# malak29/video-text-detection-system

Measured on AMD Instinct MI355X. Metric: frames/sec (detect+recognize) @720p, 1/2/4/8 MI355X; box IoU vs CPU ref, higher is better.
Workload: dtype f16

## Files before the change

video-text-detection-system_amd/csrc/conv_halo.hip:

```cpp
#include <cstdio>
#include <cstdlib>
#include "vtd_common.h"
#include "conv_kernels.h"

namespace {

struct HaloParams {
    const half_t* in;
    const half_t* wgt;
    const float* bias;
    const half_t* res;
    half_t* out;
    int n, h, w, cin, cout;
    int in_hp, in_wp, in_ring, out_hp, out_wp, out_ring, res_hp, res_wp, res_ring;
    int tiles_x, tiles_y, tiles_n, relu;
    unsigned long long* stamps;
    const half_t* in2 = nullptr;
    int in2_hp = 0, in2_wp = 0, in2_c = 0, in2_ring = 0;
    int K = 0;
    int dbg;
};

template <int N>
__device__ __forceinline__ void hl_wait_vmcnt() {
    asm volatile("s_waitcnt vmcnt(%0)" ::"n"(N) : "memory");
}

template <int BN, int TW>
__global__ __launch_bounds__((BN / 64) * 256) void conv_halo_kernel(const HaloParams p) {
    constexpr int WN = BN / 64, NW = 4 * WN, NT = NW * 64, TH = 256 / TW;
    constexpr int HWD = TW + 2, HROWS = (TH + 2) * HWD, HPIECES = (HROWS + 7) / 8, HBYTES = HPIECES * 1024;
    constexpr int HPW = (HPIECES + NW - 1) / NW;
    constexpr int HPS = (HPW + 7) / 8;
    constexpr int BSTAGE = BN * 128, BPW = BN / 8 / NW;
    constexpr int EPI_ROW = BN * 4 + 16;
    static_assert(BPW == 2, "two weight pieces per wave and K-step");
    extern __shared__ __attribute__((aligned(16))) char smem[];

    const int nchunks = p.cin >> 6;
    const int hb_stride = nchunks > 1 ? HBYTES : 0;
    char* const bring = smem + (nchunks > 1 ? 2 : 1) * HBYTES;

    const int nblk = gridDim.x, b = blockIdx.x;
    const int q8 = nblk >> 3, r8 = nblk & 7, xcd = b & 7;
    int tile = (xcd < r8 ? xcd * (q8 + 1) : r8 * (q8 + 1) + (xcd - r8) * q8) + (b >> 3);
    const int tn = tile % p.tiles_n;
    tile /= p.tiles_n;
    const int tx = tile % p.tiles_x;
    tile /= p.tiles_x;
    const int ty = tile % p.tiles_y;
    const int img = tile / p.tiles_y;
    const int y0 = ty * TH, x0 = tx * TW, n0 = tn * BN;

    const int tid = threadIdx.x, lane = tid & 63;
    const int w = __builtin_amdgcn_readfirstlane(tid >> 6);
    const int lrow = lane >> 3;
    const int K = 9 * p.cin;

    int hoff[HPW];
#pragma unroll
    for (int k = 0; k < HPW; ++k) {
        const int piece = w + k * NW;
        int row = piece * 8 + lrow;
        row = row < HROWS ? row : HROWS - 1;
        const int hy = row / HWD, hx = row - hy * HWD;
        int gy = y0 - 1 + hy + p.in_ring, gx = x0 - 1 + hx + p.in_ring;
        gy = gy < p.in_hp ? gy : p.in_hp - 1;
        gx = gx < p.in_wp ? gx : p.in_wp - 1;
        const int c_log = (lane & 7) ^ (row & 6);
        hoff[k] = ((img * p.in_hp + gy) * p.in_wp + gx) * p.cin + c_log * 8;
    }
    auto issue_halo = [&](int k, int chunk, int buf) {
        const int piece = w + k * NW;
        if (piece < HPIECES)
            __builtin_amdgcn_global_load_lds((const VTD_AS1 void*)(p.in + hoff[k] + chunk * 64),
                                             (VTD_AS3 void*)(smem + buf * hb_stride + piece * 1024), 16, 0, 0);
    };
    const half_t* bsrc[BPW];
// ... 489 lines not shown
    for (int i = 0; i < 4; ++i) bias4[i] = *(const floatx4*)(p.bias + fq * 16 + i * 4);
#pragma unroll
    for (int i = 0; i < 4; ++i) asm volatile("" : "+v"(bias4[i]));

    auto tile_coords = [&](int t, int& img, int& y0, int& x0) {
        img = t / tiles_per_img;
        const int r = t - img * tiles_per_img, ty = r / p.tiles_x;
        y0 = ty * TH;
        x0 = (r - ty * p.tiles_x) * TW;
    };
    int hrel[HPW];
    int hdst[HPW];
#pragma unroll
    for (int k = 0; k < HPW; ++k) {
        const int piece = w + 4 * k;
        int row = piece * 8 + lrow;
        row = row < HROWS ? row : HROWS - 1;
        const int hy = row / HWD, hx = row - hy * HWD;
        hrel[k] = (hy * p.in_wp + hx) * 64 + ((lane & 7) ^ (row & 6)) * 8;
        hdst[k] = piece < HPIECES ? WBYTES + piece * 1024 : WBYTES + 2 * HBYTES;
    }
    auto issue_halo = [&](int img, int y0, int x0, int buf) {
        const half_t* base = p.in + ((int64_t)(img * p.in_hp + y0 - 1 + p.in_ring) * p.in_wp + x0 - 1 + p.in_ring) * 64;
#pragma unroll
        for (int k = 0; k < HPW; ++k)
            __builtin_amdgcn_global_load_lds((const VTD_AS1 void*)(base + hrel[k]),
                                             (VTD_AS3 void*)(smem + hdst[k] + (w + 4 * k < HPIECES ? buf * HBYTES : 0)), 16, 0, 0);
    };
    int orel[4], rrel[4];
#pragma unroll
    for (int j = 0; j < 4; ++j) {
        const int m = w * 64 + j * 16 + fr;
        orel[j] = ((m / TW) * p.out_wp + (m % TW)) * 64 + fq * 16;
        rrel[j] = ((m / TW) * p.res_wp + (m % TW)) * 64 + fq * 16;
    }

    int hbase[4];
#pragma unroll
    for (int j = 0; j < 4; ++j) {
        const int m = w * 64 + j * 16 + fr;
        hbase[j] = (m / TW) * HWD + (m % TW);
    }
    const int bswz = (fr >> 1) & 7;

    auto load_res = [&](int img, int y0, int x0, half8 (&rv)[4][2]) {
        const half_t* rbase = p.res + ((int64_t)(img * p.res_hp + y0 + p.res_ring) * p.res_wp + x0 + p.res_ring) * 64;
#pragma unroll
        for (int j = 0; j < 4; ++j) {
            rv[j][0] = *(const half8*)(rbase + rrel[j]);
            rv[j][1] = *(const half8*)(rbase + rrel[j] + 8);
        }
    };

    int tile = blockIdx.x;
    if (tile >= total) return;
    int img, y0, x0;
    tile_coords(tile, img, y0, x0);
    issue_halo(img, y0, x0, 0);
    int cur = 0;
    unsigned long long acc_wait = 0, acc_loop = 0, acc_epi = 0, t_a = 0, t_b = 0, t_c = 0;
    for (; tile < total; tile += gridDim.x, cur ^= 1) {
        if (p.stamps) t_a = __builtin_amdgcn_s_memtime();
        const int ntile = tile + gridDim.x;
        int nimg = img, ny0 = y0, nx0 = x0;
        half8 rv[4][2];
        if (RES) load_res(img, y0, x0, rv);
        if (ntile < total) tile_coords(ntile, nimg, ny0, nx0);
        issue_halo(nimg, ny0, nx0, cur ^ 1);
        if (RES) hl_wait_vmcnt<HPW + 8>(); else hl_wait_vmcnt<HPW>();
        __builtin_amdgcn_s_barrier();
        if (p.stamps) t_b = __builtin_amdgcn_s_memtime();

        floatx4 acc[4][4];
#pragma unroll
        for (int i = 0; i < 4; ++i)
#pragma unroll
            for (int j = 0; j < 4; ++j) acc[i][j] = bias4[i];
        const char* hb = hbuf + cur * HBYTES;
        auto load_frags = [&](int hs, half8 (&af)[4], half8 (&bf)[4]) {
            const int tap = hs >> 1, kk = hs & 1;
            const int tapoff = (tap / 3) * HWD + (tap % 3);
#pragma unroll
            for (int j = 0; j < 4; ++j) {
                const int hrow = hbase[j] + tapoff;
                af[j] = *(const half8*)(hb + hrow * 128 + (((fq + 4 * kk) ^ (hrow & 6)) << 4));
            }
#pragma unroll
            for (int i = 0; i < 4; ++i) bf[i] = *(const half8*)(wl + tap * 8192 + (i * 16 + fr) * 128 + (((fq + 4 * kk) ^ bswz) << 4));
        };
        half8 fa[2][4], fb[2][4];
        load_frags(0, fa[0], fb[0]);
#pragma unroll
        for (int hs = 0; hs < 18; ++hs) {
            if (hs + 1 < 18) load_frags(hs + 1, fa[(hs + 1) & 1], fb[(hs + 1) & 1]);
#pragma unroll
            for (int i = 0; i < 4; ++i)
#pragma unroll
                for (int j = 0; j < 4; ++j)
                    acc[i][j] = __builtin_amdgcn_mfma_f32_16x16x32_f16(fb[hs & 1][i], fa[hs & 1][j], acc[i][j], 0, 0, 0);
            if (hs + 1 < 18) {
                __builtin_amdgcn_sched_group_barrier(0x100, 8, 0);
                __builtin_amdgcn_sched_group_barrier(0x008, 16, 0);
            }
            __builtin_amdgcn_sched_barrier(0);
        }

        if (p.stamps) {
            asm volatile("s_nop 0" ::"v"(acc[3][3][3]));
            t_c = __builtin_amdgcn_s_memtime();
        }
        half_t* obase = p.out + ((int64_t)(img * p.out_hp + y0 + p.out_ring) * p.out_wp + x0 + p.out_ring) * 64;
#pragma unroll
        for (int j = 0; j < 4; ++j)
#pragma unroll
            for (int h = 0; h < 2; ++h) {
                half8 hv;
#pragma unroll
                for (int k = 0; k < 8; ++k) {
                    float v = acc[2 * h + (k >> 2)][j][k & 3];
                    if (RES) v += (float)rv[j][h][k];
                    hv[k] = (half_t)(RELU ? fmaxf(v, 0.f) : v);
                }
                *(half8*)(obase + orel[j] + h * 8) = hv;
            }
        __builtin_amdgcn_s_barrier();
        img = nimg; y0 = ny0; x0 = nx0;
        if (p.stamps) {
            const unsigned long long t_d = __builtin_amdgcn_s_memtime();
            acc_wait += t_b - t_a; acc_loop += t_c - t_b; acc_epi += t_d - t_c;
        }
    }
    if (p.stamps && tid == 0) {
        unsigned long long* o = p.stamps + (int64_t)blockIdx.x * 4;
        o[0] = 0; o[1] = acc_wait; o[2] = acc_wait + acc_loop; o[3] = acc_wait + acc_loop + acc_epi;
    }
    hl_wait_vmcnt<0>();
}

template <int TW, bool RELU, bool RES>
__global__ __launch_bounds__(512, 1) void conv3x3_c64_duo_kernel(const HaloParams p) {
    constexpr int TH = 256 / TW, HWD = TW + 2, HROWS = (TH + 2) * HWD, HPIECES = (HROWS + 7) / 8, HBYTES = HPIECES * 1024;
    constexpr int HPW = (HPIECES + 3) / 4;
    constexpr int WBYTES = 9 * 64 * 128;
    extern __shared__ __attribute__((aligned(16))) char smem[];
    char* const wl = smem;
    char* const hbuf = smem + WBYTES;

    const int tid = threadIdx.x, lane = tid & 63;
    const int wv = __builtin_amdgcn_readfirstlane(tid >> 6);
    const int g = wv >> 2, w = wv & 3;
    const int lrow = lane >> 3, fr = lane & 15, fq = lane >> 4;
    const int tiles_per_img = p.tiles_x * p.tiles_y, total = p.n * tiles_per_img;

#pragma unroll
    for (int k = 0; k < 9; ++k) {
        const int piece = wv + 8 * k, tap = piece >> 3, row = (piece & 7) * 8 + lrow;
        const int c_log = (lane & 7) ^ ((row >> 1) & 7);
        const int cout = 16 * ((row & 15) >> 2) + 4 * (row >> 4) + (row & 3);
        __builtin_amdgcn_global_load_lds((const VTD_AS1 void*)(p.wgt + cout * 576 + tap * 64 + c_log * 8),
                                         (VTD_AS3 void*)(wl + piece * 1024), 16, 0, 0);
    }
    float* const bias_lds = (float*)(smem + WBYTES + 2 * HBYTES + 1024);
    if (tid < 64) bias_lds[tid] = p.bias[tid];

    auto tile_coords = [&](int t, int& img, int& y0, int& x0) {
        img = t / tiles_per_img;
        const int r = t - img * tiles_per_img, ty = r / p.tiles_x;
        y0 = ty * TH;
        x0 = (r - ty * p.tiles_x) * TW;
    };
    auto issue_halo = [&](int t) {
        int img, y0, x0;
        tile_coords(t, img, y0, x0);
        const half_t* base = p.in + ((int64_t)(img * p.in_hp + y0 - 1 + p.in_ring) * p.in_wp + x0 - 1 + p.in_ring) * 64;
#pragma unroll
        for (int k = 0; k < HPW; ++k) {
            const int piece = w + 4 * k;
            int row = piece * 8 + lrow;
            row = row < HROWS ? row : HROWS - 1;
            const int hy = row / HWD, hx = row - hy * HWD;
            const int hrel = (hy * p.in_wp + hx) * 64 + ((lane & 7) ^ (hx & 6)) * 8;
            const int hdst = piece < HPIECES ? WBYTES + g * HBYTES + piece * 1024 : WBYTES + 2 * HBYTES;
            __builtin_amdgcn_global_load_lds((const VTD_AS1 void*)(base + hrel), (VTD_AS3 void*)(smem + hdst), 16, 0, 0);
        }
    };
    auto px_row = [&](int j) { return (w * 64 + j * 16 + fr) / TW; };
    auto px_col = [&](int j) { return (w * 64 + j * 16 + fr) % TW; };
    const int a_lane_off = (px_row(0) * HWD + px_col(0)) * 128;
    const int b_lane_off = fr * 128;
    const int bswz = (fr >> 1) & 7;
    const char* const hb = hbuf + g * HBYTES;

    const int nq = (total - (int)blockIdx.x + (int)gridDim.x - 1) / (int)gridDim.x;
    const int nmine = (nq - g + 1) >> 1;
    const int phases = 2 * ((nq + 1) >> 1) > 2 * (nq >> 1) + 1 ? 2 * ((nq + 1) >> 1) : 2 * (nq >> 1) + 1;
#ifdef VTD_CONV_EXPERIMENT
    auto block_of = [&](int i) { return p.dbg == 1 ? (int)blockIdx.x : (int)blockIdx.x + (2 * i + g) * (int)gridDim.x; };
#else
    auto block_of = [&](int i) { return (int)blockIdx.x + (2 * i + g) * (int)gridDim.x; };
#endif

    if (nmine > 0) issue_halo(block_of(0));
    hl_wait_vmcnt<0>();
    asm volatile("s_waitcnt lgkmcnt(0)" ::: "memory");
    __builtin_amdgcn_s_barrier();

    floatx4 acc[4][4];
    half8 rv[4][2];
    for (int phase = 0; phase < phases; ++phase) {
        if ((phase & 1) == g) {
            const int i = (phase - g) >> 1;
            if (i < nmine) {
                if (RES) {
                    int img, y0, x0;
                    tile_coords(block_of(i), img, y0, x0);
                    const half_t* rbase = p.res + ((int64_t)(img * p.res_hp + y0 + p.res_ring) * p.res_wp + x0 + p.res_ring) * 64;
#pragma unroll
                    for (int j = 0; j < 4; ++j) {
                        const int rrel = (px_row(j) * p.res_wp + px_col(j)) * 64 + fq * 16;
                        rv[j][0] = *(const half8*)(rbase + rrel);
                        rv[j][1] = *(const half8*)(rbase + rrel + 8);
                    }
                }
#pragma unroll
                for (int a = 0; a < 4; ++a)
#pragma unroll
                    for (int j = 0; j < 4; ++j) acc[a][j] = *(const floatx4*)(bias_lds + fq * 16 + a * 4);
                auto load_frags = [&](int hs, half8 (&af)[4], half8 (&bf)[4]) {
                    const int tap = hs >> 1, kk = hs & 1;
                    const int tapoff = (tap / 3) * HWD + (tap % 3), dx = tap % 3;
                    const char* pa = hb + a_lane_off + tapoff * 128 + (((fq + 4 * kk) ^ ((fr + dx) & 6)) << 4);
                    const char* pb = wl + tap * 8192 + b_lane_off + (((fq + 4 * kk) ^ bswz) << 4);
#pragma unroll
                    for (int j = 0; j < 4; ++j) af[j] = *(const half8*)(pa + (TW == 16 ? j * HWD : (j >> 1) * HWD + (j & 1) * 16) * 128);
#pragma unroll
                    for (int a = 0; a < 4; ++a) bf[a] = *(const half8*)(pb + a * 2048);
                };
                half8 fa[2][4], fb[2][4];
                load_frags(0, fa[0], fb[0]);
#pragma unroll
                for (int hs = 0; hs < 18; ++hs) {
                    if (hs + 1 < 18) load_frags(hs + 1, fa[(hs + 1) & 1], fb[(hs + 1) & 1]);
#pragma unroll
                    for (int a = 0; a < 4; ++a)
#pragma unroll
                        for (int j = 0; j < 4; ++j)
                            acc[a][j] = __builtin_amdgcn_mfma_f32_16x16x32_f16(fb[hs & 1][a], fa[hs & 1][j], acc[a][j], 0, 0, 0);
                    if (hs + 1 < 18) {
                        __builtin_amdgcn_sched_group_barrier(0x100, 8, 0);
                        __builtin_amdgcn_sched_group_barrier(0x008, 16, 0);
                    }
                    __builtin_amdgcn_sched_barrier(0);
                    if (hs + 1 < 18) {
#pragma unroll
                        for (int j = 0; j < 4; ++j) asm volatile("" ::"v"(fa[(hs + 1) & 1][j]));
#pragma unroll
                        for (int a = 0; a < 4; ++a) asm volatile("" ::"v"(fb[(hs + 1) & 1][a]));
                    }
                }
            }
        } else {
            const int i = (phase - g - 1) >> 1;
            if (phase - g - 1 >= 0 && i < nmine) {
                if (i + 1 < nmine) issue_halo(block_of(i + 1));
                int img, y0, x0;
                tile_coords(block_of(i), img, y0, x0);
                half_t* obase = p.out + ((int64_t)(img * p.out_hp + y0 + p.out_ring) * p.out_wp + x0 + p.out_ring) * 64;
#pragma unroll
                for (int j = 0; j < 4; ++j)
#pragma unroll
                    for (int h = 0; h < 2; ++h) {
                        half8 hv;
#pragma unroll
                        for (int k = 0; k < 8; ++k) {
                            float v = acc[2 * h + (k >> 2)][j][k & 3];
                            if (RES) v += (float)rv[j][h][k];
                            hv[k] = (half_t)(RELU ? fmaxf(v, 0.f) : v);
                        }
                        *(half8*)(obase + (px_row(j) * p.out_wp + px_col(j)) * 64 + fq * 16 + h * 8) = hv;
                    }
            }
            hl_wait_vmcnt<0>();
        }
        __builtin_amdgcn_s_barrier();
    }
    hl_wait_vmcnt<0>();
}

template <int TW, bool RELU, bool RES>
int c64_launch(const HaloParams& p, hipStream_t stream) {
    constexpr int TH = 256 / TW, HROWS = (TH + 2) * (TW + 2), HBYTES = (HROWS + 7) / 8 * 1024;
    constexpr int lds = 9 * 64 * 128 + 2 * HBYTES + 1024 + 256;
    static_assert(lds <= 160 * 1024, "LDS budget");
    if (p.h % TH || p.w % TW) return -2205;
    static bool attr_done = false;
    if (!attr_done) {
        hipError_t e = hipFuncSetAttribute((const void*)conv3x3_c64_persistent_kernel<TW, RELU, RES>,
                                           hipFuncAttributeMaxDynamicSharedMemorySize, lds);
        if (e != hipSuccess) return -(int)e;
        attr_done = true;
    }
    const int total = p.n * p.tiles_y * p.tiles_x;
    const int grid = total < 256 ? total : 256;
    static const bool want_stamps = [] { const char* e = getenv("VTD_HALO_STAMPS"); return e && e[0] == '1'; }();
    if (want_stamps) {
        HaloParams q = p;
        unsigned long long* dev = nullptr;
        if (hipMalloc(&dev, (size_t)grid * 32) != hipSuccess) return -2204;
        q.stamps = dev;
        hipLaunchKernelGGL((conv3x3_c64_persistent_kernel<TW, RELU, RES>), dim3(grid), dim3(256), lds, stream, q);
        (void)hipStreamSynchronize(stream);
        unsigned long long* h = (unsigned long long*)malloc((size_t)grid * 32);
        (void)hipMemcpy(h, dev, (size_t)grid * 32, hipMemcpyDeviceToHost);
        double a = 0, b = 0, c = 0;
        for (int i = 0; i < grid; ++i) { a += (double)h[4 * i + 1]; b += (double)(h[4 * i + 2] - h[4 * i + 1]); c += (double)(h[4 * i + 3] - h[4 * i + 2]); }
        const double blocks = (double)total / grid;
        fprintf(stderr, "[c64 stamps] res=%d blocks/WG %.1f: per block ticks: issue+wait %.1f  K-loop %.1f  epilogue %.1f\n", (int)RES, blocks,
                a / grid / blocks, b / grid / blocks, c / grid / blocks);
        free(h);
        (void)hipFree(dev);
        return 0;
    }
    const char* duo_env = getenv("VTD_C64_DUO");
    const bool duo = !(duo_env && duo_env[0] == '0');
#ifdef VTD_CONV_EXPERIMENT
    if (duo) {
        HaloParams q = p;
        const char* d = getenv("VTD_C64_DEBUG");
        q.dbg = d ? atoi(d) : 0;
        hipError_t e = hipFuncSetAttribute((const void*)conv3x3_c64_duo_kernel<TW, RELU, RES>, hipFuncAttributeMaxDynamicSharedMemorySize, lds);
        if (e != hipSuccess) return -(int)e;
        hipLaunchKernelGGL((conv3x3_c64_duo_kernel<TW, RELU, RES>), dim3(grid), dim3(512), lds, stream, q);
        return -(int)hipGetLastError();
    }
#endif
    if (duo) {
        static bool attr_duo = false;
        if (!attr_duo) {
            hipError_t e = hipFuncSetAttribute((const void*)conv3x3_c64_duo_kernel<TW, RELU, RES>, hipFuncAttributeMaxDynamicSharedMemorySize, lds);
            if (e != hipSuccess) return -(int)e;
            attr_duo = true;
        }
        hipLaunchKernelGGL((conv3x3_c64_duo_kernel<TW, RELU, RES>), dim3(grid), dim3(512), lds, stream, p);
        return -(int)hipGetLastError();
    }
    hipLaunchKernelGGL((conv3x3_c64_persistent_kernel<TW, RELU, RES>), dim3(grid), dim3(256), lds, stream, p);
    return -(int)hipGetLastError();
}

template <int TW>
int c64_dispatch(const HaloParams& p, hipStream_t stream) {
    if (p.relu) return p.res ? c64_launch<TW, true, true>(p, stream) : c64_launch<TW, true, false>(p, stream);
    return p.res ? c64_launch<TW, false, true>(p, stream) : c64_launch<TW, false, false>(p, stream);
}

template <int BN, int TW>
// ... 24 lines not shown
        double pro = 0, loop = 0, epi = 0;
        unsigned long long t0 = ~0ull, t1 = 0;
        for (int i = 0; i < grid; ++i) {
            pro += (double)(h[4 * i + 1] - h[4 * i]); loop += (double)(h[4 * i + 2] - h[4 * i + 1]); epi += (double)(h[4 * i + 3] - h[4 * i + 2]);
            t0 = h[4 * i] < t0 ? h[4 * i] : t0; t1 = h[4 * i + 3] > t1 ? h[4 * i + 3] : t1;
        }
        fprintf(stderr, "[halo stamps] BN=%d TW=%d cin=%d cout=%d grid=%d: per-WG ticks (100 MHz) prologue %.1f  K-loop %.1f  epilogue %.1f; kernel span %llu ticks\n",
                BN, TW, p.cin, p.cout, grid, pro / grid, loop / grid, epi / grid, t1 - t0);
        free(h);
        (void)hipFree(dev);
        return 0;
    }
    hipLaunchKernelGGL((conv_halo_kernel<BN, TW>), dim3(grid), dim3((BN / 64) * 256), lds, stream, p);
    return -(int)hipGetLastError();
}

}

static bool halo_common_rules(const ConvParams& c, bool second_segment = false) {
    if (c.plist || (c.in2 && !second_segment) || c.pool_pw || c.stride != 1 || c.kw != 3 || c.K != 9 * c.in_c + (c.in2 ? 64 : 0) || (c.in_c & 63)) return false;
    if (c.cin_steps * 64 != c.in_c || c.s_step != c.in_c || c.r_step != c.in_wp * c.in_c || c.k_hi_step != 32) return false;
    if ((c.cout & 63) || c.cout != c.cout_pad || c.out_c != c.cout) return false;
    if (c.flags & ~(EPI_RELU | EPI_RESIDUAL)) return false;
    if ((c.flags & EPI_RESIDUAL) && (c.res_shift || !c.res)) return false;
    return !(c.in_y0 < 0 || c.in_x0 != c.in_y0 || c.ho <= 0 || c.wo <= 0 || c.M % (c.ho * c.wo));
}

bool vtd_conv_halo_supported(const ConvParams& c, int* bn_out, int* tw_out) {
    if (!halo_common_rules(c)) return false;
    const int h = c.ho, w = c.wo;
    auto eff = [&](int th, int tw) { return (double)h * w / ((double)((h + th - 1) / th * th) * ((w + tw - 1) / tw * tw)); };
    const double e16 = eff(16, 16), e32 = eff(8, 32);
    const int tw = e16 >= e32 ? 16 : 32;
    if ((tw == 16 ? e16 : e32) < 0.85) return false;
    *tw_out = tw;
    *bn_out = (c.cout % 128 == 0) ? 128 : 64;
    return true;
}

bool vtd_conv_halo_c64_supported(const ConvParams& c, int tw) {
    return c.in_c == 64 && c.cout == 64 && c.wo % tw == 0 && c.ho % (256 / tw) == 0;
}

int vtd_launch_conv_halo(const ConvParams& c, int bn, int tw, hipStream_t stream) {
    HaloParams p;
    p.in = c.in; p.wgt = c.wgt; p.bias = c.bias; p.res = (c.flags & EPI_RESIDUAL) ? c.res : nullptr; p.out = (half_t*)c.out;
    p.h = c.ho; p.w = c.wo; p.n = c.M / (c.ho * c.wo); p.cin = c.in_c; p.cout = c.cout;
    p.in_hp = c.in_hp; p.in_wp = c.in_wp; p.in_ring = c.in_y0 + 1;
    p.out_hp = c.out_hp; p.out_wp = c.out_wp; p.out_ring = c.out_ring;
    p.res_hp = c.res_hp; p.res_wp = c.res_wp; p.res_ring = c.res_ring;
    p.relu = (c.flags & EPI_RELU) ? 1 : 0;
    p.stamps = nullptr;
    p.dbg = 0;
    if (c.in_y0 != c.in_x0 || c.in_y0 < 0 || c.K != 9 * c.in_c || c.out_c != c.cout || p.n <= 0 || (c.in_c & 63) || (c.cout & 63) ||
        (tw != 16 && tw != 32) || c.stride != 1 || c.M != p.n * c.ho * c.wo)
        return -2201;
    if ((int64_t)p.n * c.in_hp * c.in_wp * c.in_c >= (1ll << 31)) return -2202;
    const int th = 256 / tw;
    p.tiles_x = (p.w + tw - 1) / tw; p.tiles_y = (p.h + th - 1) / th; p.tiles_n = bn > 1 ? p.cout / bn : 1;
    if (bn == 2) {
        p.tiles_n = p.cout / 64;
        return tw == 16 ? halo64_launch<16>(p, stream) : halo64_launch<32>(p, stream);
    }
    if (bn == 1) {
        if (p.cin != 64 || p.cout != 64) return -2201;
        p.tiles_n = 1;
        return tw == 16 ? c64_dispatch<16>(p, stream) : c64_dispatch<32>(p, stream);
    }
    if (bn == 64 && tw == 16) return halo_launch<64, 16>(p, stream);
    if (bn == 64 && tw == 32) return halo_launch<64, 32>(p, stream);
    if (bn == 128 && tw == 16) return halo_launch<128, 16>(p, stream);
    if (bn == 128 && tw == 32) return halo_launch<128, 32>(p, stream);
    return -2201;
}

bool vtd_conv_halo_small_supported(const ConvParams& c) {
    if (!halo_common_rules(c, true) || c.ho % 8 || c.wo % 16) return false;
    if (c.in2 && (c.in2_mul != 2 || c.in2_shr != 0 || c.cin_steps2 != 1 || c.kw2 != 1 || c.seg1_steps * 64 != 9 * c.in_c || c.in2_c < 64 || (c.in2_c & 7) ||
                  c.in2_ring < 0 || 2 * (c.ho - 1) + c.in2_ring >= c.in2_hp || 2 * (c.wo - 1) + c.in2_ring >= c.in2_wp))
        return false;
    return c.in_hp >= c.ho + c.in_y0 + 2 && c.in_wp >= c.wo + c.in_y0 + 2;
}

int vtd_launch_conv_halo_small(const ConvParams& c, hipStream_t stream) {
    if (c.ho <= 0 || c.wo <= 0) return -2201;
    HaloParams p;
    p.in = c.in; p.wgt = c.wgt; p.bias = c.bias; p.res = (c.flags & EPI_RESIDUAL) ? c.res : nullptr; p.out = (half_t*)c.out;
    p.h = c.ho; p.w = c.wo; p.n = c.M / (c.ho * c.wo); p.cin = c.in_c; p.cout = c.cout;
    p.in_hp = c.in_hp; p.in_wp = c.in_wp; p.in_ring = c.in_y0 + 1;
    p.out_hp = c.out_hp; p.out_wp = c.out_wp; p.out_ring = c.out_ring;
    p.res_hp = c.res_hp; p.res_wp = c.res_wp; p.res_ring = c.res_ring;
    p.relu = (c.flags & EPI_RELU) ? 1 : 0;
    p.stamps = nullptr;
    p.dbg = 0;
    p.K = c.K;
    if (c.in2) { p.in2 = c.in2; p.in2_hp = c.in2_hp; p.in2_wp = c.in2_wp; p.in2_c = c.in2_c; p.in2_ring = c.in2_ring; }
    if (c.in_y0 != c.in_x0 || c.in_y0 < 0 || c.K != 9 * c.in_c + (c.in2 ? 64 : 0) || c.out_c != c.cout || p.n <= 0 || (c.in_c & 63) || (c.cout & 63) ||
        c.stride != 1 || c.M != p.n * c.ho * c.wo || (c.ho & 7) || (c.wo & 15) || ((c.flags & EPI_RESIDUAL) && !c.res) || c.plist)
        return -2201;
    if (c.in2 && (c.in2_mul != 2 || c.in2_shr != 0 || c.in2_c < 64 || (c.in2_c & 7) || c.in2_ring < 0 || 2 * (c.ho - 1) + c.in2_ring >= c.in2_hp ||
                  2 * (c.wo - 1) + c.in2_ring >= c.in2_wp || (int64_t)p.n * c.in2_hp * c.in2_wp * c.in2_c >= (1ll << 31)))
        return -2201;
    if (c.in_hp < c.ho + p.in_ring + 1 || c.in_wp < c.wo + p.in_ring + 1 || c.out_ring < 0 || c.out_hp < c.ho + c.out_ring || c.out_wp < c.wo + c.out_ring ||
        (p.res && (c.res_ring < 0 || c.res_hp < c.ho + c.res_ring || c.res_wp < c.wo + c.res_ring)))
        return -2201;
    if ((int64_t)p.n * c.in_hp * c.in_wp * c.in_c >= (1ll << 31)) return -2202;
    p.tiles_x = p.w / 16; p.tiles_y = p.h / 8; p.tiles_n = p.cout / 64;
    hipLaunchKernelGGL(conv_halo_small_kernel, dim3(p.n * p.tiles_y * p.tiles_x * p.tiles_n), dim3(256), 0, stream, p);
    return -(int)hipGetLastError();
}
```

video-text-detection-system_amd/csrc/conv_select.cpp:

```cpp
#include "conv_select.h"
#include <algorithm>
#include <cstdio>
#include <cstdlib>
#include <cstring>

namespace vtd {
static void fill_conv_params(const ConvOp& c, int n, ConvParams& p) {
    std::memset(&p, 0, sizeof(p));
    p.in = c.in.ptr; p.wgt = c.w; p.k_hi_step = c.k_hi_step; p.cin_steps = c.cin_steps; p.kw = c.kw; p.s_step = c.s_step; p.r_step = c.r_step; p.bias = c.bias;
    p.res = c.has_res ? c.res.ptr : nullptr;
    p.out = (c.flags & (EPI_OUT_F32 | EPI_OUT_F16)) ? c.out_f32 : (void*)c.out.ptr;
    p.M = n * c.ho * c.wo; p.K = c.K; p.cout = c.cout; p.cout_pad = c.cout_pad;
    p.ho = c.ho; p.wo = c.wo;
    p.in_hp = c.in.hp; p.in_wp = c.in.wp; p.in_c = c.in.c; p.in_y0 = c.in_y0; p.in_x0 = c.in_x0; p.stride = c.stride;
    p.out_hp = c.out.hp; p.out_wp = c.out.wp; p.out_c = c.out.c; p.out_ring = c.out.ring;
    p.res_hp = c.res.hp; p.res_wp = c.res.wp; p.res_ring = c.res.ring; p.res_shift = c.res_shift;
    p.ps_cout = c.ps_cout; p.flags = c.flags; p.ldc = c.ldc;
    p.seg_cols = c.seg_cols;
    for (int i = 0; i < 3; ++i) { p.seg_out[i] = c.seg_out[i]; p.seg_ldc[i] = c.seg_ldc[i]; }
    p.head_w = c.head_w; p.head_b = c.head_b; p.prob_out = (float*)c.out_f32;
    if (c.plist) {
        p.plist = c.plist; p.tile_combo = c.tile_combo; p.tiles_per_img = c.tiles_per_img;
        p.plist_b = c.plist_b; p.tile_combo_b = c.tile_combo_b; p.tiles_per_img_b = c.tiles_per_img_b;
        p.in2 = c.in2.ptr; p.in2_hp = c.in2.hp; p.in2_wp = c.in2.wp; p.in2_c = c.in2.c; p.in2_ring = c.in2.ring;
        p.seg1_steps = c.seg1_steps; p.cin_steps2 = c.cin_steps2; p.kw2 = c.kw2; p.s_step2 = c.s_step2; p.r_step2 = c.r_step2;
        p.bias_tab = c.bias_tab; p.img_h = c.img_h; p.img_w = c.img_w;
        p.M = n * c.tiles_per_img * 128;
    }
    p.pool_pw = c.pool_pw;
    if (c.dual) {
        p.in2 = c.in2.ptr; p.in2_hp = c.in2.hp; p.in2_wp = c.in2.wp; p.in2_c = c.in2.c; p.in2_ring = c.in2.ring;
        p.in2_mul = c.in2_mul; p.in2_shr = c.in2_shr;
        p.seg1_steps = c.seg1_steps; p.cin_steps2 = c.cin_steps2; p.kw2 = 1; p.s_step2 = 0; p.r_step2 = 0;
    }
}

static bool env_is(const char* name, char v) { const char* e = std::getenv(name); return e && e[0] == v; }
static bool halo_enabled() { return !env_is("VTD_HALO_CONV", '0'); }
static bool autotune_enabled() { return !env_is("VTD_AUTOTUNE", '0'); }

static bool halo_valid(const ConvParams& p, bool c64) {
    int bn = 0, tw = 0;
    return vtd_conv_halo_supported(p, &bn, &tw) && (!c64 || vtd_conv_halo_c64_supported(p, tw));
}
static int launch_halo(const ConvParams& p, int bn, hipStream_t s) {
    int hbn = 0, tw = 0;
    return vtd_conv_halo_supported(p, &hbn, &tw) ? vtd_launch_conv_halo(p, bn ? bn : hbn, tw, s) : ERR_GEOMETRY;
}
static bool head_entry_valid(const ConvOp& c, const ConvParams& p) { return p.plist && c.he_steps && c.tile_combo_border; }

static const ConvCandidate kCandidates[] = {
    {kHeadEntryHaloCfg, "head_entry_halo", head_entry_valid,
     [](const ConvOp& c, const ConvParams& p, hipStream_t s) { return vtd_launch_head_entry_halo(p, c.he_steps, c.he_nsteps, 0, s); }, true, true, 0, 4, 2},
    {kHeadEntryHalo256Cfg, "head_entry_halo256", head_entry_valid,
     [](const ConvOp& c, const ConvParams& p, hipStream_t s) { return vtd_launch_head_entry_halo(p, c.he_steps, c.he_nsteps, 1, s); }, true, true, 0, 4, 2},
#ifdef VTD_EXPERIMENTAL_CANDIDATES
    {kHeadEntryPairCfg, "head_entry_pair", [](const ConvOp& c, const ConvParams& p) { return head_entry_valid(c, p) && c.hp_half_steps; },
     [](const ConvOp& c, const ConvParams& p, hipStream_t s) { return vtd_launch_head_entry_pair(p, c.hp_half_steps, c.hp_plan, c.hp_nh, s); }, true, true, 0, 4, 2},
    {kHeadEntryHalfCfg, "head_entry_half", [](const ConvOp& c, const ConvParams& p) { return head_entry_valid(c, p) && c.hh_sched; },
     [](const ConvOp& c, const ConvParams& p, hipStream_t s) { return vtd_launch_head_entry_half(p, c.hh_sched, c.he_nsteps, s); }, true, true, 0, 4, 2},
#endif
    {kPointwiseCfg, "pointwise128", [](const ConvOp&, const ConvParams& p) { return vtd_pointwise128_supported(p); },
     [](const ConvOp&, const ConvParams& p, hipStream_t s) { return vtd_launch_pointwise128(p, s); }, false, false, 0, 3, 1},
    {kHaloCfg, "conv_halo", [](const ConvOp&, const ConvParams& p) { return halo_valid(p, false); },
     [](const ConvOp&, const ConvParams& p, hipStream_t s) { return launch_halo(p, 0, s); }, false, true, 0, 3, 1},
    {kHaloC64Cfg, "conv_halo_c64_persistent", [](const ConvOp&, const ConvParams& p) { return halo_valid(p, true); },
     [](const ConvOp&, const ConvParams& p, hipStream_t s) { return launch_halo(p, 1, s); }, false, true, '2', 3, 1},
    {kHalo64Cfg, "conv_halo64", [](const ConvOp&, const ConvParams& p) { return halo_valid(p, false); },
     [](const ConvOp&, const ConvParams& p, hipStream_t s) { return launch_halo(p, 2, s); }, false, true, '3', 3, 1},
    {kHaloSmallCfg, "conv_halo_small", [](const ConvOp&, const ConvParams& p) { return vtd_conv_halo_small_supported(p); },
     [](const ConvOp&, const ConvParams& p, hipStream_t s) { return vtd_launch_conv_halo_small(p, s); }, false, true, '4', 3, 1},
};

const ConvCandidate* find_conv_candidate(int id) {
    for (const ConvCandidate& row : kCandidates)
        if (row.id == id) return &row;
    return nullptr;
}

static int pick_tile_height(const ConvParams& p, int table_cfg) {
    if (const char* e = std::getenv("VTD_TILE_HEIGHT_MODEL"); e && e[0] == '0') return table_cfg;
    if (std::getenv("VTD_FORCE_CONV_CFG")) return table_cfg;
// ... 192 lines not shown
```

video-text-detection-system_amd/csrc/conv_select.h:

```cpp
#pragma once
#include <map>
#include <string>
#include "conv_kernels.h"

namespace vtd {
enum : int {
    ERR_ARG = -1100, ERR_UNKNOWN_KEY = -1101, ERR_SHAPE = -1102, ERR_MISSING_KEY = -1103,
    ERR_NOT_FINALIZED = -1104, ERR_BATCH = -1105, ERR_GEOMETRY = -1106, ERR_CAPACITY = -1107,
};

struct ConvOp {
    TensorDesc in, out, res;
    bool has_res = false;
    half_t* w = nullptr;
    half_t* w_panel = nullptr;
    float* bias = nullptr;
    int k_hi_step = 32, cin_steps = 1, kw = 1, s_step = 0, r_step = 0;
    int K = 0, cout = 0, cout_pad = 0, stride = 1, in_y0 = 0, in_x0 = 0, flags = 0, ps_cout = 0, res_shift = 0;
    int ho = 0, wo = 0;
    int64_t macs_per_image = 0;
    void* out_f32 = nullptr;
    int ldc = 0;
    int seg_cols = 0;
    void* seg_out[3] = {nullptr, nullptr, nullptr};
    int seg_ldc[3] = {0, 0, 0};
    const float* head_w = nullptr;
    float head_b = 0.f;
    const uint32_t* plist = nullptr;
    const int* tile_combo = nullptr;
    const uint32_t* plist_b = nullptr;
    const int* tile_combo_border = nullptr;
    int tiles_border = 0;
    const int* he_steps = nullptr;
    int he_nsteps = 0;
    const int* hh_sched = nullptr;
    const int* hp_half_steps = nullptr;
    const int* hp_plan = nullptr;
    int hp_nh = 0;
    const int* tile_combo_b = nullptr;
    int tiles_per_img_b = 0;
    int tiles_per_img = 0, seg1_steps = 0, cin_steps2 = 0, kw2 = 0, s_step2 = 0, r_step2 = 0, img_h = 0, img_w = 0;
    TensorDesc in2;
    const float* bias_tab = nullptr;
    bool dual = false;
    int in2_mul = 1, in2_shr = 0;
    int pool_pw = 0;
};

static const int kHaloCfg = 100;
static const int kHaloC64Cfg = 101;
static const int kHeadEntryHaloCfg = 102;
static const int kHeadEntryHalo256Cfg = 103;
static const int kHalo64Cfg = 104;
static const int kHeadEntryPairCfg = 105;
static const int kPointwiseCfg = 106;
static const int kHeadEntryHalfCfg = 107;
static const int kHaloSmallCfg = 108;

struct ConvCandidate {
    int id;
    const char* name;
    bool (*valid)(const ConvOp&, const ConvParams&);
    int (*launch)(const ConvOp&, const ConvParams&, hipStream_t);
    bool needs_border;
    bool halo_switch;
    char force_halo;
    int reps, rounds;
};
const ConvCandidate* find_conv_candidate(int id);
int launch_conv_op(const ConvOp& c, int n, hipStream_t s, int cfg = -1, float* prob_out = nullptr);
int launch_border_tiles(const ConvOp& c, int n, hipStream_t s);

struct TuningTable {
    std::map<std::string, int> tuning;
    bool tuning_measured = false;
};
int choose_config(TuningTable* m, const ConvOp& c, int n, hipStream_t s, int* cfg);
int set_tuning_text(TuningTable* m, const char* text);
int64_t get_tuning_text(const TuningTable* m, char* buf, int64_t cap);
int batch_bucket(int n, int cap);
}
```

video-text-detection-system_amd/csrc/vtd_api.cpp:

```cpp
#include <algorithm>
#include <cmath>
#include <cstdio>
#include <cstdlib>
#include <cstring>
#include <map>
#include <memory>
#include <string>
#include <vector>

#include "../../include/vtd.h"
#include "vtd_common.h"
#include "conv_select.h"

int vtd_launch_preprocess(const uint8_t* frames, int n, int H, int W, half_t* out, const int* xb, const int* xk, int ksx,
                          const int* yb, const int* yk, int ksy, int max_rows, hipStream_t stream);
int vtd_preprocess_max_rows(const int* yb);
int vtd_preprocess_path(int W, int ksx, int ksy, int max_rows, int* lds_bytes);
int vtd_launch_nchw_to_input(const float* x, half_t* out, int n, hipStream_t stream);
int vtd_launch_maxpool(const TensorDesc& in, const TensorDesc& out, int n, int kh, int kw, int sh, int sw, int pad_h, int pad_w,
                       hipStream_t stream);
void vtd_stem_pool_pack_weights(const float* w_folded, half_t* packed);
int vtd_launch_stem_pool(const TensorDesc& in, const TensorDesc& out, const half_t* w_packed, const float* bias, int n, hipStream_t stream);
void vtd_head_tail_pack_w1(const half_t* w1_gemm, half_t* packed);
void vtd_head_tail_pack_w2(const float* w2, half_t* packed);
// ... 854 lines not shown
    for (int br = 0; br < 2; ++br) {
        const std::string hp = branch[br];
        TensorDesc h1;
        if ((rc = new_tensor(160, 160, 64, h1))) return rc;
        Fold f1, f2;
        ConvOp c1;
        if (fuse) {
            if ((rc = build_classed_head_entry(d, c1, tapsC[0], last, h1, hp))) return rc;
        } else {
            if ((rc = fold_bn(d, hp + "1", hp + "0.bias", 64, f1))) return rc;
            if ((rc = build_conv(d, c1, p2, h1, hp + "0.weight", f1, 256, 64, 3, 3, 1, 1, EPI_RELU))) return rc;
        }
        if ((rc = fold_bn(d, hp + "4", hp + "3.bias", 64, f2))) return rc;
        ConvOp c2;
        TensorDesc h2 = make_desc(B, 320, 320, 64, 1, 1);
        std::vector<half_t> w1_host;
        if ((rc = build_convt(d, c2, h1, h2, hp + "3.weight", f2, 64, 64, EPI_RELU, &w1_host))) return rc;
        auto w6 = d->get(hp + "6.weight", 64 * 4), b6 = d->get(hp + "6.bias", 1);
        if (!w6 || !b6) return ERR_MISSING_KEY;
        std::vector<float> wf(4 * 64);
        for (int blk = 0; blk < 4; ++blk)
            for (int ci = 0; ci < 64; ++ci) wf[blk * 64 + ci] = (*w6)[ci * 4 + blk];
        float* wdev = nullptr;
        if ((rc = upload(d->arena, wf.data(), wf.size() * sizeof(float), (void**)&wdev))) return rc;
        c2.flags = EPI_HEAD_FINAL;
        c2.head_w = wdev;
        c2.head_b = (*b6)[0];
        Op o1, o2;
        o1.kind = Op::CONV; o1.conv = c1; o1.final_slot = br;
        o2.kind = Op::FINAL; o2.conv = c2; o2.final_slot = br;
        if (d->head_tail_kernel) {
            std::vector<half_t> p1((size_t)4 * 4 * 2 * 64 * 8), p2((size_t)2 * 64 * 8);
            vtd_head_tail_pack_w1(w1_host.data(), p1.data());
            vtd_head_tail_pack_w2(wf.data(), p2.data());
            if ((rc = upload(d->arena, p1.data(), p1.size() * sizeof(half_t), (void**)&o2.htw1))) return rc;
            if ((rc = upload(d->arena, p2.data(), p2.size() * sizeof(half_t), (void**)&o2.htw2))) return rc;
            o2.kind = Op::HEADTAIL;
        }
        d->ops.push_back(o1);
        if (fuse) {
            Op ob;
            ob.kind = Op::BORDER; ob.conv = c1; ob.final_slot = br;
            ob.conv.macs_per_image = (int64_t)c1.tiles_border * 128 * 64 * c1.K;
            d->ops.push_back(ob);
        }
        d->ops.push_back(o2);
        if (br == 0) {
            const int64_t px = (int64_t)160 * 160;
            const int64_t ref_entry = fuse ? px * 256 * tapsC[0].c + px * 256 * 2304 + px * 64 * 2304 : c1.macs_per_image;
            d->macs += ref_entry + c2.macs_per_image + (int64_t)320 * 320 * 4 * 64;
            d->taps["head1"] = h1;
        }
    }
    return 0;
}

static int read_tensor_nchw(const TensorDesc& t, int n, int creal, float* host_out, hipStream_t stream) {
    hipError_t e = hipStreamSynchronize(stream);
    if (e != hipSuccess) return -(int)e;
    std::vector<half_t> tmp((size_t)n * t.hp * t.wp * t.c);
    e = hipMemcpy(tmp.data(), t.ptr, tmp.size() * sizeof(half_t), hipMemcpyDeviceToHost);
    if (e != hipSuccess) return -(int)e;
    for (int img = 0; img < n; ++img)
        for (int c = 0; c < creal; ++c)
            for (int y = 0; y < t.h; ++y)
                for (int x = 0; x < t.w; ++x)
                    host_out[(((size_t)img * creal + c) * t.h + y) * t.w + x] =
                        (float)tmp[(((size_t)img * t.hp + y + t.ring) * t.wp + x + t.ring) * t.c + c];
    return 0;
}

static int build_linear(ModelBase* d, ConvOp& op, const TensorDesc& in, const std::vector<float>& W, const std::vector<float>& bias,
                        int N, int K, void* out_f32, int ldc, int out_flag = EPI_OUT_F32) {
    if (in.c != K || (K & 63) || (int)W.size() != N * K || (int)bias.size() != N || (ldc & 3) || ldc < N) return ERR_GEOMETRY;
    const int cout_pad = (N + 63) / 64 * 64;
    std::vector<half_t> wp((size_t)cout_pad * K, (half_t)0.f);
    for (size_t i = 0; i < (size_t)N * K; ++i) wp[i] = (half_t)W[i];
    std::vector<float> b(cout_pad, 0.f);
    for (int i = 0; i < N; ++i) b[i] = bias[i];
    op.cin_steps = K / 64; op.kw = 1; op.s_step = 0; op.r_step = 0; op.k_hi_step = 32;
    int rc;
    if ((rc = upload(d->arena, wp.data(), wp.size() * sizeof(half_t), (void**)&op.w))) return rc;
    if ((rc = upload(d->arena, b.data(), b.size() * sizeof(float), (void**)&op.bias))) return rc;
    op.in = in; op.out = in; op.K = K; op.cout = N; op.cout_pad = cout_pad; op.stride = 1;
    op.in_y0 = in.ring; op.in_x0 = in.ring; op.flags = out_flag; op.ho = in.h; op.wo = in.w;
    op.out_f32 = out_f32; op.ldc = ldc;
    op.macs_per_image = (int64_t)in.h * in.w * N * K;
    return 0;
}

static bool known_detector_key(const std::string& k) {
    return k.rfind("backbone.", 0) == 0 || k.rfind("fpn.", 0) == 0 || k.rfind("head.", 0) == 0;
}

static int get_pre_tables(vtd_detector* d, int H, int W, PreTables& out) {
    auto key = std::make_pair(H, W);
    auto it = d->pre.find(key);
    if (it != d->pre.end()) {
        out = it->second;
        return 0;
    }
    ResampleAxis ax = pillow_axis(W, 640), ay = pillow_axis(H, 640);
    PreTables t;
    t.ksx = ax.ksize; t.ksy = ay.ksize;
    t.max_rows = vtd_preprocess_max_rows(ay.bounds.data());
    int rc;
// ... 877 lines not shown
```

video-text-detection-system_amd/csrc/vtd_common.h:

```cpp
#pragma once
#include <hip/hip_runtime.h>
#include <stdint.h>

typedef _Float16 half_t;
typedef half_t half8 __attribute__((ext_vector_type(8)));
typedef half_t half4 __attribute__((ext_vector_type(4)));
typedef half_t half2v __attribute__((ext_vector_type(2)));
typedef float floatx4 __attribute__((ext_vector_type(4)));

#define VTD_AS1 __attribute__((address_space(1)))
#define VTD_AS3 __attribute__((address_space(3)))

struct TensorDesc {
    half_t* ptr;
    int n, h, w, c;
    int ring;
    int hp, wp;
};

static inline __host__ __device__ int64_t tensor_elems(const TensorDesc& t) {
    return (int64_t)t.n * t.hp * t.wp * t.c;
}

enum : int {
// ... 1 lines not shown
    EPI_RESIDUAL = 2,
    EPI_PIXEL_SHUFFLE = 4,
    EPI_OUT_F32 = 8,
    EPI_OUT_F16 = 32,
    EPI_GELU = 64,
    EPI_HEAD_FINAL = 16,
};

struct ConvParams {
    const half_t* in;
    const half_t* wgt;
    int cin_steps, kw, s_step, r_step;
    int k_hi_step;
    const float* bias;
    const half_t* res;
    void* out;
    int M;
    int K;
    int cout;
    int cout_pad;
    int ho, wo;
    int in_hp, in_wp, in_c;
    int in_y0, in_x0;
    int stride;
    int out_hp, out_wp, out_c, out_ring;
    int res_hp, res_wp, res_ring, res_shift;
    int ps_cout;
    int flags;
    int dbg;
    int ldc;
    int seg_cols;
    void* seg_out[3];
    int seg_ldc[3];
    int epi_direct;
    int pool_pw, pool_log2, pool_wq, pool_hqwq;
    uint64_t magic_wo, magic_howo;
    int magic_ok;
    const uint32_t* plist;
    const int* tile_combo;
    const uint32_t* plist_b;
    const int* tile_combo_b;
    int tiles_per_img_b;
    int tiles_per_img;
    const half_t* in2;
    int in2_hp, in2_wp, in2_c, in2_ring;
    int in2_mul, in2_shr;
    int seg1_steps;
    int cin_steps2, kw2, s_step2, r_step2;
    const float* bias_tab;
    int img_h, img_w;
    const float* head_w;
    float head_b;
    float* prob_out;
};

#define VTD_HIP_CHECK(expr)                                   \
    do {                                                      \
        hipError_t _e = (expr);                               \
        if (_e != hipSuccess) return -(int)_e;                \
    } while (0)
```

Before: 12660.

## Replace static tile striding with atomic dynamic tile claiming in 3x3 c64 convs

The persistent 3x3 64-channel conv kernels now take their next tiles from a per-op global atomic counter instead of a fixed blockIdx + k*gridDim stride. Claims are issued early in the compute phase and the result is passed to the other waves through LDS control words, so halo prefetch can still overlap. The last workgroup to finish resets the counter. The intent is to balance load when workgroups run at uneven speeds, at the cost of atomics, extra LDS syncs and more complex termination logic in the dual-group kernel.

```diff
diff --git a/video-text-detection-system_amd/csrc/conv_halo.hip b/video-text-detection-system_amd/csrc/conv_halo.hip
--- a/video-text-detection-system_amd/csrc/conv_halo.hip
+++ b/video-text-detection-system_amd/csrc/conv_halo.hip
@@ -18,12 +18,31 @@
     const half_t* in2 = nullptr;
     int in2_hp = 0, in2_wp = 0, in2_c = 0, in2_ring = 0;
     int K = 0;
+    unsigned int* claim = nullptr;
     int dbg;
 };
 
 template <int N>
 __device__ __forceinline__ void hl_wait_vmcnt() {
     asm volatile("s_waitcnt vmcnt(%0)" ::"n"(N) : "memory");
+}
+
+__device__ __forceinline__ unsigned int claim_block(unsigned int* counter) {
+    unsigned int zero = 0;
+    asm volatile("" : "+v"(zero));
+    return __hip_atomic_fetch_add(counter + zero, 1u, __ATOMIC_RELAXED, __HIP_MEMORY_SCOPE_AGENT);
+}
+__device__ __forceinline__ void claim_leave(unsigned int* claim, unsigned int workgroups) {
+    if (__hip_atomic_fetch_add(claim + 1, 1u, __ATOMIC_RELAXED, __HIP_MEMORY_SCOPE_AGENT) == workgroups - 1) {
+        __hip_atomic_store(claim, 0u, __ATOMIC_RELAXED, __HIP_MEMORY_SCOPE_AGENT);
+        __hip_atomic_store(claim + 1, 0u, __ATOMIC_RELAXED, __HIP_MEMORY_SCOPE_AGENT);
+    }
+}
+constexpr int kClaimCtlBytes = 64;
+__device__ __forceinline__ int claim_ctl_read(const volatile int* word) {
+    int v;
+    asm volatile("ds_read_b32 %0, %1\n\ts_waitcnt lgkmcnt(0)" : "=v"(v) : "v"((unsigned int)(uintptr_t)(const VTD_AS3 void*)word) : "memory");
+    return __builtin_amdgcn_readfirstlane(v);
 }
 
 template <int BN, int TW>
@@ -619,16 +638,18 @@
         }
     };
 
+    unsigned int* const claim = p.claim;
+    volatile int* const ctl = (volatile int*)(smem + WBYTES + 2 * HBYTES + 1024 + 256);
     int tile = blockIdx.x;
     if (tile >= total) return;
+    int ntile = tile + (int)gridDim.x;
     int img, y0, x0;
     tile_coords(tile, img, y0, x0);
     issue_halo(img, y0, x0, 0);
     int cur = 0;
     unsigned long long acc_wait = 0, acc_loop = 0, acc_epi = 0, t_a = 0, t_b = 0, t_c = 0;
-    for (; tile < total; tile += gridDim.x, cur ^= 1) {
+    for (; tile < total; cur ^= 1) {
         if (p.stamps) t_a = __builtin_amdgcn_s_memtime();
-        const int ntile = tile + gridDim.x;
         int nimg = img, ny0 = y0, nx0 = x0;
         half8 rv[4][2];
         if (RES) load_res(img, y0, x0, rv);
@@ -637,6 +658,9 @@
         if (RES) hl_wait_vmcnt<HPW + 8>(); else hl_wait_vmcnt<HPW>();
         __builtin_amdgcn_s_barrier();
         if (p.stamps) t_b = __builtin_amdgcn_s_memtime();
+        const bool claimer = claim && w == 0;
+        unsigned int got = 0;
+        if (claimer && ntile < total && lane == 0) got = claim_block(claim);
 
         floatx4 acc[4][4];
 #pragma unroll
@@ -672,6 +696,10 @@
             __builtin_amdgcn_sched_barrier(0);
         }
 
+        if (claimer) {
+            if (lane == 0) ctl[0] = (ntile < total && got < (unsigned int)total) ? (int)got + 2 * (int)gridDim.x : total;
+            asm volatile("s_waitcnt lgkmcnt(0)" ::: "memory");
+        }
         if (p.stamps) {
             asm volatile("s_nop 0" ::"v"(acc[3][3][3]));
             t_c = __builtin_amdgcn_s_memtime();
@@ -691,6 +719,9 @@
                 *(half8*)(obase + orel[j] + h * 8) = hv;
             }
         __builtin_amdgcn_s_barrier();
+        asm volatile("" ::: "memory");
+        const int nntile = claim ? claim_ctl_read(ctl) : (ntile < total ? ntile + (int)gridDim.x : total);
+        tile = ntile; ntile = nntile;
         img = nimg; y0 = ny0; x0 = nx0;
         if (p.stamps) {
             const unsigned long long t_d = __builtin_amdgcn_s_memtime();
@@ -702,6 +733,7 @@
         o[0] = 0; o[1] = acc_wait; o[2] = acc_wait + acc_loop; o[3] = acc_wait + acc_loop + acc_epi;
     }
     hl_wait_vmcnt<0>();
+    if (claim && tid == 0) claim_leave(claim, gridDim.x);
 }
 
 template <int TW, bool RELU, bool RES>
@@ -758,29 +790,37 @@
     const int bswz = (fr >> 1) & 7;
     const char* const hb = hbuf + g * HBYTES;
 
-    const int nq = (total - (int)blockIdx.x + (int)gridDim.x - 1) / (int)gridDim.x;
-    const int nmine = (nq - g + 1) >> 1;
+    const int G = (int)gridDim.x;
+    unsigned int* const claim = p.claim;
+    volatile int* const ctl = (volatile int*)(smem + WBYTES + 2 * HBYTES + 1024 + 256);
+    const int nq = (total - (int)blockIdx.x + G - 1) / G;
     const int phases = 2 * ((nq + 1) >> 1) > 2 * (nq >> 1) + 1 ? 2 * ((nq + 1) >> 1) : 2 * (nq >> 1) + 1;
 #ifdef VTD_CONV_EXPERIMENT
-    auto block_of = [&](int i) { return p.dbg == 1 ? (int)blockIdx.x : (int)blockIdx.x + (2 * i + g) * (int)gridDim.x; };
+    auto where = [&](int blk) { return p.dbg == 1 ? (int)blockIdx.x : blk; };
 #else
-    auto block_of = [&](int i) { return (int)blockIdx.x + (2 * i + g) * (int)gridDim.x; };
+    auto where = [&](int blk) { return blk; };
 #endif
-
-    if (nmine > 0) issue_halo(block_of(0));
+    int cur = (int)blockIdx.x + g * G;
+    bool pending = false;
+
+    if (cur < total) issue_halo(where(cur));
     hl_wait_vmcnt<0>();
     asm volatile("s_waitcnt lgkmcnt(0)" ::: "memory");
     __builtin_amdgcn_s_barrier();
 
     floatx4 acc[4][4];
     half8 rv[4][2];
-    for (int phase = 0; phase < phases; ++phase) {
+    int held0 = 1, held1 = 0;
+    for (int phase = 0;; ++phase) {
+        bool hold;
         if ((phase & 1) == g) {
-            const int i = (phase - g) >> 1;
-            if (i < nmine) {
+            if (cur < total) {
+                const bool claimer = claim && w == 0;
+                unsigned int got = 0;
+                if (claimer && lane == 0) got = claim_block(claim);
                 if (RES) {
                     int img, y0, x0;
-                    tile_coords(block_of(i), img, y0, x0);
+                    tile_coords(where(cur), img, y0, x0);
                     const half_t* rbase = p.res + ((int64_t)(img * p.res_hp + y0 + p.res_ring) * p.res_wp + x0 + p.res_ring) * 64;
 #pragma unroll
                     for (int j = 0; j < 4; ++j) {
@@ -825,13 +865,16 @@
                         for (int a = 0; a < 4; ++a) asm volatile("" ::"v"(fb[(hs + 1) & 1][a]));
                     }
                 }
-            }
+                pending = true;
+                if (claimer && lane == 0) ctl[g] = got < (unsigned int)total ? (int)got + 2 * G : total;
+            }
+            hold = pending;
         } else {
-            const int i = (phase - g - 1) >> 1;
-            if (phase - g - 1 >= 0 && i < nmine) {
-                if (i + 1 < nmine) issue_halo(block_of(i + 1));
+            if (pending) {
+                const int next = claim ? claim_ctl_read(ctl + g) : (cur + 2 * G < total ? cur + 2 * G : total);
+                if (next < total) issue_halo(where(next));
                 int img, y0, x0;
-                tile_coords(block_of(i), img, y0, x0);
+                tile_coords(where(cur), img, y0, x0);
                 half_t* obase = p.out + ((int64_t)(img * p.out_hp + y0 + p.out_ring) * p.out_wp + x0 + p.out_ring) * 64;
 #pragma unroll
                 for (int j = 0; j < 4; ++j)
@@ -846,20 +889,39 @@
                         }
                         *(half8*)(obase + (px_row(j) * p.out_wp + px_col(j)) * 64 + fq * 16 + h * 8) = hv;
                     }
-            }
+                cur = next;
+                pending = false;
+            }
+            hold = cur < total;
             hl_wait_vmcnt<0>();
         }
+        if (claim) {
+            if (w == 0 && lane == 0) ctl[2 + 2 * (phase & 1) + g] = hold;
+            asm volatile("s_waitcnt lgkmcnt(0)" ::: "memory");
+        }
         __builtin_amdgcn_s_barrier();
+        if (claim) {
+            asm volatile("" ::: "memory");
+            if (!__builtin_amdgcn_readfirstlane(held0 | held1)) break;
+            held0 = ctl[2 + 2 * (phase & 1)];
+            held1 = ctl[3 + 2 * (phase & 1)];
+        } else if (phase + 1 >= phases) {
+            break;
+        }
     }
     hl_wait_vmcnt<0>();
+    if (claim && tid == 0) claim_leave(claim, gridDim.x);
 }
 
 template <int TW, bool RELU, bool RES>
-int c64_launch(const HaloParams& p, hipStream_t stream) {
+int c64_launch(const HaloParams& p_in, hipStream_t stream) {
     constexpr int TH = 256 / TW, HROWS = (TH + 2) * (TW + 2), HBYTES = (HROWS + 7) / 8 * 1024;
-    constexpr int lds = 9 * 64 * 128 + 2 * HBYTES + 1024 + 256;
+    constexpr int lds = 9 * 64 * 128 + 2 * HBYTES + 1024 + 256 + kClaimCtlBytes;
     static_assert(lds <= 160 * 1024, "LDS budget");
-    if (p.h % TH || p.w % TW) return -2205;
+    if (p_in.h % TH || p_in.w % TW) return -2205;
+    static const bool claim_on = [] { const char* e = getenv("VTD_TILE_CLAIM"); return !(e && e[0] == '0'); }();
+    HaloParams p = p_in;
+    if (!claim_on) p.claim = nullptr;
     static bool attr_done = false;
     if (!attr_done) {
         hipError_t e = hipFuncSetAttribute((const void*)conv3x3_c64_persistent_kernel<TW, RELU, RES>,
@@ -868,7 +930,11 @@
         attr_done = true;
     }
     const int total = p.n * p.tiles_y * p.tiles_x;
-    const int grid = total < 256 ? total : 256;
+    int grid = total < 256 ? total : 256;
+    if (const char* cap = getenv("VTD_C64_GRID_CAP")) {
+        const int g = atoi(cap);
+        if (g > 0 && g < grid) grid = g;
+    }
     static const bool want_stamps = [] { const char* e = getenv("VTD_HALO_STAMPS"); return e && e[0] == '1'; }();
     if (want_stamps) {
         HaloParams q = p;
@@ -999,6 +1065,7 @@
     p.relu = (c.flags & EPI_RELU) ? 1 : 0;
     p.stamps = nullptr;
     p.dbg = 0;
+    p.claim = c.claim;
     if (c.in_y0 != c.in_x0 || c.in_y0 < 0 || c.K != 9 * c.in_c || c.out_c != c.cout || p.n <= 0 || (c.in_c & 63) || (c.cout & 63) ||
         (tw != 16 && tw != 32) || c.stride != 1 || c.M != p.n * c.ho * c.wo)
         return -2201;
@@ -1019,6 +1086,18 @@
     if (bn == 128 && tw == 16) return halo_launch<128, 16>(p, stream);
     if (bn == 128 && tw == 32) return halo_launch<128, 32>(p, stream);
     return -2201;
+}
+
+extern "C" int vtd_conv_c64_single(const void* in, const void* wgt, const float* bias, const void* res, void* out, int n, int h, int w, int relu,
+                                   unsigned int* claim, void* stream) {
+    if (!in || !wgt || !bias || !out || n <= 0 || h <= 0 || w <= 0 || (h & 15) || (w & 15)) return -2201;
+    ConvParams c = {};
+    c.in = (const half_t*)in; c.wgt = (const half_t*)wgt; c.bias = bias; c.res = (const half_t*)res; c.out = out;
+    c.M = n * h * w; c.K = 576; c.cout = c.cout_pad = c.out_c = c.in_c = 64; c.ho = h; c.wo = w; c.stride = 1;
+    c.in_hp = c.out_hp = c.res_hp = h + 2; c.in_wp = c.out_wp = c.res_wp = w + 2; c.out_ring = c.res_ring = 1;
+    c.flags = (relu ? EPI_RELU : 0) | (res ? EPI_RESIDUAL : 0);
+    c.claim = claim;
+    return vtd_launch_conv_halo(c, 1, 16, (hipStream_t)stream);
 }
 
 bool vtd_conv_halo_small_supported(const ConvParams& c) {
diff --git a/video-text-detection-system_amd/csrc/conv_select.cpp b/video-text-detection-system_amd/csrc/conv_select.cpp
--- a/video-text-detection-system_amd/csrc/conv_select.cpp
+++ b/video-text-detection-system_amd/csrc/conv_select.cpp
@@ -28,6 +28,7 @@
         p.M = n * c.tiles_per_img * 128;
     }
     p.pool_pw = c.pool_pw;
+    p.claim = c.claim;
     if (c.dual) {
         p.in2 = c.in2.ptr; p.in2_hp = c.in2.hp; p.in2_wp = c.in2.wp; p.in2_c = c.in2.c; p.in2_ring = c.in2.ring;
         p.in2_mul = c.in2_mul; p.in2_shr = c.in2_shr;
diff --git a/video-text-detection-system_amd/csrc/conv_select.h b/video-text-detection-system_amd/csrc/conv_select.h
--- a/video-text-detection-system_amd/csrc/conv_select.h
+++ b/video-text-detection-system_amd/csrc/conv_select.h
@@ -45,6 +45,7 @@
     bool dual = false;
     int in2_mul = 1, in2_shr = 0;
     int pool_pw = 0;
+    unsigned int* claim = nullptr;
 };
 
 static const int kHaloCfg = 100;
diff --git a/video-text-detection-system_amd/csrc/vtd_api.cpp b/video-text-detection-system_amd/csrc/vtd_api.cpp
--- a/video-text-detection-system_amd/csrc/vtd_api.cpp
+++ b/video-text-detection-system_amd/csrc/vtd_api.cpp
@@ -930,6 +930,17 @@
             d->taps["head1"] = h1;
         }
     }
+    auto c64_slot = [](const Op& o) {
+        return o.kind == Op::CONV && !o.conv.plist && o.conv.in.c == 64 && o.conv.cout == 64 && o.conv.K == 576 && o.conv.stride == 1;
+    };
+    size_t slots = 0;
+    for (const Op& o : d->ops) slots += c64_slot(o);
+    if (slots) {
+        char* lines = nullptr;
+        if ((rc = d->arena.alloc((void**)&lines, slots * 128, true))) return rc;
+        for (Op& o : d->ops)
+            if (c64_slot(o)) { o.conv.claim = (unsigned int*)lines; lines += 128; }
+    }
     return 0;
 }
 
diff --git a/video-text-detection-system_amd/csrc/vtd_common.h b/video-text-detection-system_amd/csrc/vtd_common.h
--- a/video-text-detection-system_amd/csrc/vtd_common.h
+++ b/video-text-detection-system_amd/csrc/vtd_common.h
@@ -77,6 +77,7 @@
     const float* head_w;
     float head_b;
     float* prob_out;
+    unsigned int* claim = nullptr;
 };
 
 #define VTD_HIP_CHECK(expr)                                   \
```

New measurement: 12790, median of 6. No clear change (+1.0%).
